# kepengxu/PGTFormer

Measured on NVIDIA H100. Metric: clips_per_s, higher is better.
Workload: dtype bf16

## Files before the change

include/pgt_b200.h:

```cpp
#ifndef PGT_B200_H_
#define PGT_B200_H_

#include <stdint.h>

#ifdef __cplusplus
extern "C" {
#endif

typedef enum pgt_status {
  PGT_OK = 0,
  PGT_ERR_INVALID = -1,
  PGT_ERR_CUDA = -2,
  PGT_ERR_UNSUPPORTED = -3,
  PGT_ERR_DRIVER = -4
} pgt_status;

enum { PGT_BF16 = 0, PGT_F32 = 1 };
enum { PGT_ACT_NONE = 0, PGT_ACT_GELU = 1, PGT_ACT_SILU = 2, PGT_ACT_LRELU02 = 3, PGT_ACT_RELU = 4,
       PGT_ACT_SIGMOID = 5 };
enum { PGT_EPI_PLAIN = 0,
       PGT_EPI_SFT = 1 };
enum { PGT_OUT_NHWC = 0, PGT_OUT_NCHW = 1 };
enum { PGT_EPI_FLAG_RELU_AFTER_RESIDUAL = 1 };

// ... 37 lines not shown

int pgt_conv_out_gn(const void* x, int F, int H, int W, int Cin, int ldx, const float* gn_ab, const void* Wp, int ldw,
                    int Cout, const float* bias, float* out, void* stream);
int pgt_conv_out_gn_act(const void* x, int F, int H, int W, int Cin, int ldx, const float* gn_ab, const void* Wp, int ldw,
                        int Cout, const float* bias, float* out, int silu, void* stream);

int pgt_conv_up2x_bf16(const void* x, int F, int Hin, int Win, int Cin, int ldx, const void* Wp4, int ldw,
                       int Cout, const pgt_epilogue* ep, void* stream);

int pgt_conv_rgb_bf16(const float* x_nchw, int F, int H, int W, int ksize, int stride, int pad, const float* mean3,
                      const float* std3, const void* Wp, int ldw, int Cout, const float* bias, int act, void* out,
                      int ldo, float* gn_stats, void* stream);

int64_t pgt_groupnorm_ws_floats(int F, int HW, int C);
int pgt_conv_tiles_per_frame(int Hin, int Win, int Cout, int ksize, int stride, int pad_lo);
int pgt_conv_tiles_exact(int Hin, int Win, int Cout, int ksize, int stride, int pad_lo);
int pgt_groupnorm_apply_stats(const void* x, int ldx, int F, int HW, int C, const float* gamma, const float* beta,
                              float eps, int apply_silu, void* y, int ldy, const float* stats, int chunks_per_frame,
                              float* ws, void* stream);

int pgt_groupnorm_ab(const void* x, int ldx, int F, int HW, int C, const float* gamma, const float* beta, float eps,
                     const float* stats, int chunks_per_frame, float* ws, float* ab, void* stream);
int pgt_groupnorm_silu(const void* x, int ldx, int F, int HW, int C, const float* gamma, const float* beta,
                       float eps, int apply_silu, void* y, int ldy, float* ws, void* stream);

int pgt_layernorm(const void* x, int ldx, int x_dtype, int T, int C, const float* gamma, const float* beta,
                  float eps, void* y, int ldy, const void* pos, int ldpos, void* y2, int ldy2, void* stream);

int pgt_ln_linear_bf16(const void* x, int ldx, int T, int C, const float* ln_g, const float* ln_b, float eps,
                       const void* W, int ldw, int N, const float* bias, void* out, int ldo, void* stream);

int pgt_swin_mlp_bf16(const void* x, int ldx, int T, int C, const float* ln_g, const float* ln_b, float eps,
                      const void* W1, const float* b1, const void* W2, const float* b2, void* out, int ldo,
                      float* gn_stats, void* stream);

int pgt_window_attention(const void* qkv, int ldqkv, int clips, int H, int W, int C, int heads, int shift,
                         const float* bias_tab, void* out, int ldo, void* stream);

int pgt_window_attention_tc(const void* qkv, int ldqkv, int clips, int H, int W, int C, int heads, int shift,
                            const void* tab, void* out, int ldo, void* stream);

int pgt_window3d_attention(const void* qkv, int ldqkv, const void* pad_qkv, int B, int D, int H, int W, int C, int heads,
                           int wd, int wh, int ww, int sd, int sh, int sw, const float* bias, void* out, int ldo,
                           void* stream);

int pgt_mha_fwd(const void* q, int ldq, const void* k, int ldk, const void* v, int ldv, int clips, int L,
                int heads, int d, void* out, int ldo, void* stream);

int pgt_argmax_gather(const float* logits, int T, int K, const float* codebook, int E, const int64_t* idx_in,
                      int64_t* idx, void* quant, int ldq, int quant_dtype, void* stream);
int pgt_l2_argmin(const float* z, int T, int E, const float* codebook, int K, int64_t* idx, float* quant,
                  void* stream);
int pgt_codebook_pack(const float* codebook, int K, int E, void* cb_bf16, float* cb_norm, void* stream);
int64_t pgt_l2_argmin_ws_ints(int T);
int pgt_l2_argmin_tc(const float* z, int T, int E, const float* codebook, const void* cb_bf16, const float* cb_norm,
                     int K, int64_t* idx, float* quant, int32_t* workspace, void* stream);
int64_t pgt_l2_argmin_split_ws_ints(int T, int splits);
int pgt_l2_argmin_tc_split(const float* z, int T, int E, const float* codebook, const void* cb_bf16, const float* cb_norm,
                           int K, int splits, int64_t* idx, float* quant, int32_t* workspace, void* stream);

int pgt_soft_codes(const float* z, int T, int E, const float* codebook, const float* cb_norm, int K, float temp,
                   float* out, int ldo, void* stream);
int pgt_sample_codes(const float* p, int T, int K, int ldp, const int64_t* seed, int64_t* idx, void* stream);

int pgt_rq_residual(const float* r_in, float* r_out, const int64_t* idx, int T, int E, const float* codebook_d,
                    float* agg, int first, void* stream);
int pgt_rq_embed(const int64_t* idx, long long ldi, long long ldd, int T, int d0, int d1, const float* codebooks,
// ... 35 lines not shown
```

pgtformer_b200/_lib.py:

```python
import ctypes
import os
from ctypes import POINTER, Structure, c_char_p, c_float, c_int, c_int32, c_int64, c_void_p

HERE = os.path.dirname(os.path.abspath(__file__))
LIB_PATH = os.path.join(HERE, 'lib', 'libpgt_b200.so')

BF16, F32 = 0, 1
ACT_NONE, ACT_GELU, ACT_SILU, ACT_LRELU02, ACT_RELU, ACT_SIGMOID = 0, 1, 2, 3, 4, 5
EPI_PLAIN, EPI_SFT = 0, 1
OUT_NHWC, OUT_NCHW = 0, 1


class Epilogue(Structure):
    _fields_ = [('bias', c_void_p), ('act', c_int32), ('mode', c_int32), ('residual', c_void_p),
                ('ldr', c_int32), ('res_dtype', c_int32), ('aux', c_void_p), ('ldaux', c_int32),
                ('sft_w', c_float), ('out', c_void_p), ('ldo', c_int32), ('out_dtype', c_int32),
                ('out_layout', c_int32), ('flags', c_int32), ('gn_stats', c_void_p), ('sft_wf', c_void_p)]


SIGNATURES = {
    'pgt_strerror': (c_char_p, [c_int]),
    'pgt_last_cuda_error': (c_char_p, []),
    'pgt_version': (c_int, []),
    'pgt_launch_count': (c_int64, []),
    'pgt_reset_launch_count': (None, []),
    'pgt_tmap_cache_stats': (None, [c_void_p, c_void_p]),
    'pgt_profile_begin': (c_int, []),
    'pgt_profile_end': (c_int, [c_void_p, c_void_p, c_void_p]),
    'pgt_profile_end_csv': (c_int, [c_char_p, c_void_p, c_void_p, c_void_p]),
    'pgt_linear_bf16': (c_int, [c_void_p, c_int, c_void_p, c_int, c_int, c_int, c_int, POINTER(Epilogue), c_void_p]),
    'pgt_conv_bf16': (c_int, [c_void_p, c_int, c_int, c_int, c_int, c_int, c_void_p, c_int, c_int, c_int, c_int,
                              c_int, POINTER(Epilogue), c_void_p]),
    'pgt_conv_out_gn': (c_int, [c_void_p, c_int, c_int, c_int, c_int, c_int, c_void_p, c_void_p, c_int, c_int, c_void_p,
                                c_void_p, c_void_p]),
    'pgt_conv_out_gn_act': (c_int, [c_void_p, c_int, c_int, c_int, c_int, c_int, c_void_p, c_void_p, c_int, c_int,
                                    c_void_p, c_void_p, c_int, c_void_p]),
    'pgt_groupnorm_ab': (c_int, [c_void_p, c_int, c_int, c_int, c_int, c_void_p, c_void_p, c_float, c_void_p, c_int,
                                 c_void_p, c_void_p, c_void_p]),
    'pgt_conv_up2x_bf16': (c_int, [c_void_p, c_int, c_int, c_int, c_int, c_int, c_void_p, c_int, c_int,
                                   POINTER(Epilogue), c_void_p]),
    'pgt_conv_rgb_bf16': (c_int, [c_void_p, c_int, c_int, c_int, c_int, c_int, c_int, c_void_p, c_void_p, c_void_p, c_int,
                                  c_int, c_void_p, c_int, c_void_p, c_int, c_void_p, c_void_p]),
    'pgt_groupnorm_ws_floats': (c_int64, [c_int, c_int, c_int]),
    'pgt_conv_tiles_per_frame': (c_int, [c_int, c_int, c_int, c_int, c_int, c_int]),
    'pgt_conv_tiles_exact': (c_int, [c_int, c_int, c_int, c_int, c_int, c_int]),
    'pgt_groupnorm_apply_stats': (c_int, [c_void_p, c_int, c_int, c_int, c_int, c_void_p, c_void_p, c_float, c_int,
                                          c_void_p, c_int, c_void_p, c_int, c_void_p, c_void_p]),
    'pgt_groupnorm_silu': (c_int, [c_void_p, c_int, c_int, c_int, c_int, c_void_p, c_void_p, c_float, c_int,
                                   c_void_p, c_int, c_void_p, c_void_p]),
    'pgt_layernorm': (c_int, [c_void_p, c_int, c_int, c_int, c_int, c_void_p, c_void_p, c_float, c_void_p, c_int,
                              c_void_p, c_int, c_void_p, c_int, c_void_p]),
    'pgt_ln_linear_bf16': (c_int, [c_void_p, c_int, c_int, c_int, c_void_p, c_void_p, c_float, c_void_p, c_int, c_int,
                                   c_void_p, c_void_p, c_int, c_void_p]),
    'pgt_swin_mlp_bf16': (c_int, [c_void_p, c_int, c_int, c_int, c_void_p, c_void_p, c_float, c_void_p, c_void_p, c_void_p,
                                  c_void_p, c_void_p, c_int, c_void_p, c_void_p]),
    'pgt_window_attention': (c_int, [c_void_p, c_int, c_int, c_int, c_int, c_int, c_int, c_int, c_void_p, c_void_p,
                                     c_int, c_void_p]),
    'pgt_window_attention_tc': (c_int, [c_void_p, c_int, c_int, c_int, c_int, c_int, c_int, c_int, c_void_p, c_void_p,
                                        c_int, c_void_p]),
    'pgt_window3d_attention': (c_int, [c_void_p, c_int, c_void_p, c_int, c_int, c_int, c_int, c_int, c_int, c_int, c_int,
                                       c_int, c_int, c_int, c_int, c_void_p, c_void_p, c_int, c_void_p]),
    'pgt_mha_fwd': (c_int, [c_void_p, c_int, c_void_p, c_int, c_void_p, c_int, c_int, c_int, c_int, c_int, c_void_p,
                            c_int, c_void_p]),
    'pgt_argmax_gather': (c_int, [c_void_p, c_int, c_int, c_void_p, c_int, c_void_p, c_void_p, c_void_p, c_int,
                                  c_int, c_void_p]),
    'pgt_l2_argmin': (c_int, [c_void_p, c_int, c_int, c_void_p, c_int, c_void_p, c_void_p, c_void_p]),
    'pgt_codebook_pack': (c_int, [c_void_p, c_int, c_int, c_void_p, c_void_p, c_void_p]),
    'pgt_l2_argmin_ws_ints': (c_int64, [c_int]),
    'pgt_l2_argmin_tc': (c_int, [c_void_p, c_int, c_int, c_void_p, c_void_p, c_void_p, c_int, c_void_p, c_void_p,
                                 c_void_p, c_void_p]),
    'pgt_l2_argmin_split_ws_ints': (c_int64, [c_int, c_int]),
    'pgt_l2_argmin_tc_split': (c_int, [c_void_p, c_int, c_int, c_void_p, c_void_p, c_void_p, c_int, c_int, c_void_p,
                                       c_void_p, c_void_p, c_void_p]),
    'pgt_soft_codes': (c_int, [c_void_p, c_int, c_int, c_void_p, c_void_p, c_int, c_float, c_void_p, c_int, c_void_p]),
    'pgt_sample_codes': (c_int, [c_void_p, c_int, c_int, c_int, c_void_p, c_void_p, c_void_p]),
    'pgt_rq_residual': (c_int, [c_void_p, c_void_p, c_void_p, c_int, c_int, c_void_p, c_void_p, c_int, c_void_p]),
    'pgt_rq_embed': (c_int, [c_void_p, c_int64, c_int64, c_int, c_int, c_int, c_void_p, c_int64, c_int, c_void_p, c_int,
                             c_int, c_void_p]),
    'pgt_vq_stats_ws_doubles': (c_int64, [c_int, c_int]),
    'pgt_vq_stats': (c_int, [c_void_p, c_int, c_int, c_int, c_void_p, c_int, c_void_p, c_float, c_void_p, c_void_p,
                             c_void_p, c_void_p, c_void_p, c_void_p, c_void_p, c_void_p, c_void_p]),
    'pgt_adain': (c_int, [c_void_p, c_int, c_int, c_void_p, c_int, c_int, c_int, c_int, c_float, c_void_p, c_int,
                          c_void_p]),
    'pgt_adain_frames': (c_int, [c_void_p, c_int, c_int, c_void_p, c_int, c_int, c_int, c_int, c_float, c_void_p,
                                 c_void_p, c_int, c_void_p]),
    'pgt_maxpool3x3s2': (c_int, [c_void_p, c_int, c_int, c_int, c_int, c_int, c_void_p, c_int, c_void_p]),
    'pgt_global_avgpool': (c_int, [c_void_p, c_int, c_int, c_int, c_int, c_void_p, c_int, c_void_p]),
    'pgt_channel_affine': (c_int, [c_void_p, c_int, c_int, c_int, c_int, c_void_p, c_int, c_int, c_void_p, c_int,
# ... 46 lines not shown
```

pgtformer_b200/csrc/swin_mlp.cu:

```cuda
#include <cudaTypedefs.h>

#include "common.cuh"
#include "tmap.cuh"
#include "ptx.cuh"
#include "epi_common.cuh"

namespace pgt {

constexpr int SM_C = 256;
constexpr int SM_BM = 128;
constexpr int SM_SUB = SM_BM * 128;
constexpr int SM_WST = 3;
constexpr int SM_WBYTES = SM_C * 128;
constexpr int SM_THREADS = 320;
constexpr int SM_XLD = 68;
constexpr int SM_XCH = SM_BM * SM_XLD * 4;
constexpr int SM_SMEM = 4 * SM_SUB  + SM_WST * SM_WBYTES + SM_XCH + 128 * 8  + 256;
static_assert(SM_SMEM <= 232448, "swin_mlp smem budget");

struct SwinMlpParams {
  int T, m_tiles;
  const float* ln_g;
  const float* ln_b;
  float eps;
  const float* b1;
  const float* b2;
  float* gn_stats;
};

struct SmBars {
  uint64_t x_full, res_full, acc2_done, out_ready;
};

__device__ __forceinline__ void swin_mlp_compute(const SwinMlpParams& p, uint8_t* sX, uint8_t* sW, float* xacc, float2* xln,
                                                 SmBars* bar, uint64_t* w_full, uint64_t* w_empty, int warp, int lane) {
  const int wg = warp >> 2, w = warp & 3;
  const int half = w >> 1;
  const int rl = (w & 1) * 32 + lane;
  const int r = wg * 64 + rl;
  const int quad = r >> 5;
  const int bar_id = 1 + wg;
  float* xw = xacc + wg * 64 * SM_XLD;
  const float* xrow = xw + rl * SM_XLD;
  const uint32_t a_rows = smem_u32(sX) + wg * 64 * 128;
  int st = 0;
  uint32_t ph = 0;
  uint32_t par = 0;
  float acc[SM_C / 2];

  auto gemm = [&]() {
    int prev = -1;
    for (int kb = 0; kb < 4; ++kb) {
      mbar_wait(&w_full[st], ph);
      const uint64_t da = wgmma_desc_k_sw128(a_rows + kb * SM_SUB);
      const uint64_t db = wgmma_desc_k_sw128(smem_u32(sW) + st * SM_WBYTES);
      wgmma_fence();
#pragma unroll
      for (int k = 0; k < 4; ++k) wgmma_bf16<SM_C>(acc, da + 2 * k, db + 2 * k, (kb | k) != 0 ? 1u : 0u);
      wgmma_commit();
      wgmma_wait<1>();
      if (prev >= 0) { __syncwarp(); if (lane == 0) mbar_arrive(&w_empty[prev]); }
      prev = st;
      if (++st == SM_WST) { st = 0; ph ^= 1; }
    }
    wgmma_wait<0>();
    __syncwarp();
    if (lane == 0) mbar_arrive(&w_empty[prev]);
  };
  auto exchange = [&](auto gc, uint32_t (&v)[32]) {
    constexpr int G = decltype(gc)::value;
    named_bar_sync(bar_id, 128);
    acc_to_smem<64 * G, 64>(acc, xw, SM_XLD, w, lane);
    named_bar_sync(bar_id, 128);
    smem_row_32(xrow + half * 32, v);
  };

  for (int tile = blockIdx.x; tile < p.m_tiles; tile += gridDim.x, par ^= 1) {
    mbar_wait(&bar->x_full, par);
    float s = 0.f, q = 0.f;
#pragma unroll
    for (int sub = 0; sub < 2; ++sub) {
      const uint8_t* src = sX + (half * 2 + sub) * SM_SUB + r * 128;
#pragma unroll
      for (int c = 0; c < 8; ++c) {
        const uint4 u = *reinterpret_cast<const uint4*>(src + ((c ^ (r & 7)) << 4));
        const float2 a = unpack_bf16x2(u.x), b = unpack_bf16x2(u.y), cc = unpack_bf16x2(u.z), d = unpack_bf16x2(u.w);
        s += (a.x + a.y) + (b.x + b.y) + (cc.x + cc.y) + (d.x + d.y);
        q += a.x * a.x + a.y * a.y + b.x * b.x + b.y * b.y + cc.x * cc.x + cc.y * cc.y + d.x * d.x + d.y * d.y;
      }
    }
    if (half == 0) xln[r] = make_float2(s, q);
    named_bar_sync(bar_id, 128);
    if (half == 1) {
      const float2 o = xln[r];
      s += o.x; q += o.y;
      xln[r] = make_float2(s, q);
    }
    named_bar_sync(bar_id, 128);
    if (half == 0) {
      const float2 o = xln[r];
      s = o.x; q = o.y;
    }
    const float mean = s * (1.f / SM_C);
    const float var = fmaxf(q * (1.f / SM_C) - mean * mean, 0.f);
    const float rstd = rsqrtf(var + p.eps);
    const float nm = -mean * rstd;
#pragma unroll
    for (int sub = 0; sub < 2; ++sub) {
      const int kb = half * 2 + sub;
      uint8_t* row = sX + kb * SM_SUB + r * 128;
#pragma unroll
      for (int c = 0; c < 8; ++c) {
        uint4* ptr = reinterpret_cast<uint4*>(row + ((c ^ (r & 7)) << 4));
        const uint4 u = *ptr;
        const float2 a = unpack_bf16x2(u.x), b = unpack_bf16x2(u.y), cc = unpack_bf16x2(u.z), d = unpack_bf16x2(u.w);
        const float v[8] = {a.x, a.y, b.x, b.y, cc.x, cc.y, d.x, d.y};
        float y[8];
        if (p.ln_g != nullptr) {
          const int col = kb * 64 + c * 8;
          const float4 g0 = __ldg(reinterpret_cast<const float4*>(p.ln_g + col)), g1 = __ldg(reinterpret_cast<const float4*>(p.ln_g + col + 4));
          const float4 e0 = __ldg(reinterpret_cast<const float4*>(p.ln_b + col)), e1 = __ldg(reinterpret_cast<const float4*>(p.ln_b + col + 4));
          const float gg[8] = {g0.x, g0.y, g0.z, g0.w, g1.x, g1.y, g1.z, g1.w};
          const float ee[8] = {e0.x, e0.y, e0.z, e0.w, e1.x, e1.y, e1.z, e1.w};
#pragma unroll
          for (int j = 0; j < 8; ++j) y[j] = fmaf(fmaf(v[j], rstd, nm), gg[j], ee[j]);
        } else {
#pragma unroll
          for (int j = 0; j < 8; ++j) y[j] = fmaf(v[j], rstd, nm);
        }
        uint4 o;
        o.x = pack_bf16x2(y[0], y[1]); o.y = pack_bf16x2(y[2], y[3]);
        o.z = pack_bf16x2(y[4], y[5]); o.w = pack_bf16x2(y[6], y[7]);
        *ptr = o;
      }
    }
    fence_proxy_async();
    named_bar_sync(bar_id, 128);
    gemm();
    static_for<0, SM_C / 64>([&](auto gc) {
      constexpr int G = decltype(gc)::value;
      uint32_t v[32];
      exchange(gc, v);
      const int c0 = G * 64 + half * 32;
      const float4* b4 = reinterpret_cast<const float4*>(p.b1 + c0);
      uint8_t* dst = sX + G * SM_SUB + r * 128;
      const int ch0 = half * 4;
#pragma unroll
      for (int i = 0; i < 4; ++i) {
        const float4 ba = __ldg(b4 + 2 * i), bb = __ldg(b4 + 2 * i + 1);
        uint4 o;
        o.x = pack_bf16x2(gelu_erf(__uint_as_float(v[8 * i + 0]) + ba.x), gelu_erf(__uint_as_float(v[8 * i + 1]) + ba.y));
        o.y = pack_bf16x2(gelu_erf(__uint_as_float(v[8 * i + 2]) + ba.z), gelu_erf(__uint_as_float(v[8 * i + 3]) + ba.w));
        o.z = pack_bf16x2(gelu_erf(__uint_as_float(v[8 * i + 4]) + bb.x), gelu_erf(__uint_as_float(v[8 * i + 5]) + bb.y));
        o.w = pack_bf16x2(gelu_erf(__uint_as_float(v[8 * i + 6]) + bb.z), gelu_erf(__uint_as_float(v[8 * i + 7]) + bb.w));
        *reinterpret_cast<uint4*>(dst + (((ch0 + i) ^ (r & 7)) << 4)) = o;
      }
    });
    fence_proxy_async();
    named_bar_sync(bar_id, 128);
    gemm();
    __syncwarp();
    if (lane == 0) mbar_arrive(&bar->acc2_done);
    mbar_wait(&bar->res_full, par);
    static_for<0, SM_C / 64>([&](auto gc) {
      constexpr int G = decltype(gc)::value;
      uint32_t v[32];
      exchange(gc, v);
      const int c0 = G * 64 + half * 32;
      float f[32];
      const float4* b4 = reinterpret_cast<const float4*>(p.b2 + c0);
      uint8_t* row = sX + G * SM_SUB + r * 128;
      const int ch0 = half * 4;
#pragma unroll
      for (int i = 0; i < 4; ++i) {
        const float4 ba = __ldg(b4 + 2 * i), bb = __ldg(b4 + 2 * i + 1);
        uint4* dst = reinterpret_cast<uint4*>(row + (((ch0 + i) ^ (r & 7)) << 4));
        const uint4 u = *dst;
        const float2 a = unpack_bf16x2(u.x), b = unpack_bf16x2(u.y), cc = unpack_bf16x2(u.z), d = unpack_bf16x2(u.w);
        f[8 * i + 0] = __uint_as_float(v[8 * i + 0]) + ba.x + a.x;  f[8 * i + 1] = __uint_as_float(v[8 * i + 1]) + ba.y + a.y;
        f[8 * i + 2] = __uint_as_float(v[8 * i + 2]) + ba.z + b.x;  f[8 * i + 3] = __uint_as_float(v[8 * i + 3]) + ba.w + b.y;
        f[8 * i + 4] = __uint_as_float(v[8 * i + 4]) + bb.x + cc.x; f[8 * i + 5] = __uint_as_float(v[8 * i + 5]) + bb.y + cc.y;
        f[8 * i + 6] = __uint_as_float(v[8 * i + 6]) + bb.z + d.x;  f[8 * i + 7] = __uint_as_float(v[8 * i + 7]) + bb.w + d.y;
        uint4 o;
        o.x = pack_bf16x2(f[8 * i + 0], f[8 * i + 1]); o.y = pack_bf16x2(f[8 * i + 2], f[8 * i + 3]);
        o.z = pack_bf16x2(f[8 * i + 4], f[8 * i + 5]); o.w = pack_bf16x2(f[8 * i + 6], f[8 * i + 7]);
        *dst = o;
      }
      if (p.gn_stats != nullptr)
        gn_chunk_stats<8>(f, p.gn_stats + (((size_t)tile * 4 + quad) * 32 + c0 / 8) * 2, 0, lane);
    });
    fence_proxy_async();
    mbar_arrive(&bar->out_ready);
  }
}

__global__ void __launch_bounds__(SM_THREADS, 1)
swin_mlp_kernel(const __grid_constant__ CUtensorMap tmX, const __grid_constant__ CUtensorMap tmO,
                const __grid_constant__ CUtensorMap tmW1, const __grid_constant__ CUtensorMap tmW2,
                const SwinMlpParams p) {
  extern __shared__ __align__(1024) uint8_t smem[];
  if ((smem_u32(smem) & 1023u) != 0) __trap();
  uint8_t* sX = smem;
  uint8_t* sW = smem + 4 * SM_SUB;
  float* xacc = reinterpret_cast<float*>(sW + SM_WST * SM_WBYTES);
  float2* xln = reinterpret_cast<float2*>(sW + SM_WST * SM_WBYTES + SM_XCH);
  SmBars* bar = reinterpret_cast<SmBars*>(xln + 128);
  uint64_t* w_full = reinterpret_cast<uint64_t*>(bar + 1);
  uint64_t* w_empty = w_full + SM_WST;

  const int warp = threadIdx.x >> 5, lane = threadIdx.x & 31;
  if (warp == 8 && lane == 0) {
    tma_prefetch_desc(&tmX); tma_prefetch_desc(&tmO); tma_prefetch_desc(&tmW1); tma_prefetch_desc(&tmW2);
    mbar_init(&bar->x_full, 1); mbar_init(&bar->res_full, 1);
    mbar_init(&bar->acc2_done, 8); mbar_init(&bar->out_ready, 256);
    for (int i = 0; i < SM_WST; ++i) { mbar_init(&w_full[i], 1); mbar_init(&w_empty[i], 8); }
    fence_barrier_init();
  }
  __syncthreads();

  if (warp == 8) {
    int st = 0;
    uint32_t ph = 0;
    for (int tile = blockIdx.x; tile < p.m_tiles; tile += gridDim.x) {
      for (int gemm = 0; gemm < 2; ++gemm) {
        for (int kb = 0; kb < 4; ++kb) {
          mbar_wait(&w_empty[st], ph ^ 1);
          if (elect_one()) {
            mbar_arrive_expect_tx(&w_full[st], SM_WBYTES);
            tma_load_2d(sW + st * SM_WBYTES, gemm == 0 ? &tmW1 : &tmW2, &w_full[st], kb * 64, 0);
          }
          __syncwarp();
          if (++st == SM_WST) { st = 0; ph ^= 1; }
        }
      }
    }
  } else if (warp == 9) {
    uint32_t par = 0;
    for (int tile = blockIdx.x; tile < p.m_tiles; tile += gridDim.x, par ^= 1) {
      if (lane == 0) {
        mbar_arrive_expect_tx(&bar->x_full, 4 * SM_SUB);
        for (int kb = 0; kb < 4; ++kb) tma_load_2d(sX + kb * SM_SUB, &tmX, &bar->x_full, kb * 64, tile * SM_BM);
      }
      __syncwarp();
      mbar_wait(&bar->acc2_done, par);
      if (lane == 0) {
        mbar_arrive_expect_tx(&bar->res_full, 4 * SM_SUB);
        for (int kb = 0; kb < 4; ++kb) tma_load_2d(sX + kb * SM_SUB, &tmX, &bar->res_full, kb * 64, tile * SM_BM);
      }
      __syncwarp();
      mbar_wait(&bar->out_ready, par);
      if (lane == 0) {
        for (int kb = 0; kb < 4; ++kb) tma_store_2d(&tmO, sX + kb * SM_SUB, kb * 64, tile * SM_BM);
        bulk_commit();
        bulk_wait_read<0>();
      }
      __syncwarp();
    }
    if (lane == 0) bulk_wait0();
  } else {
    swin_mlp_compute(p, sX, sW, xacc, xln, bar, w_full, w_empty, warp, lane);

  }
}

static int enc2d(CUtensorMap* map, const void* base, int ld, long long rows, int cols, int box_rows) {
  return tmap_rows_bf16(map, base, ld, rows, cols, box_rows);
}

}

using namespace pgt;

extern "C" int pgt_swin_mlp_bf16(const void* x, int ldx, int T, int C, const float* ln_g, const float* ln_b, float eps,
                                 const void* W1, const float* b1, const void* W2, const float* b2, void* out, int ldo,
                                 float* gn_stats, void* stream) {
  PGT_CHECK_ARG(x && out && W1 && W2 && b1 && b2 && T > 0 && ((ln_g == nullptr) == (ln_b == nullptr)));
  if (C != SM_C) return PGT_ERR_UNSUPPORTED;
  auto al = [](const void* q) { return (reinterpret_cast<uintptr_t>(q) & 15) == 0; };
  PGT_CHECK_ARG(al(x) && al(out) && al(W1) && al(W2) && ldx % 8 == 0 && ldo % 8 == 0);
  CUtensorMap tx, to, t1, t2;
  int rc = enc2d(&tx, x, ldx, T, C, SM_BM);
  if (rc == PGT_OK) rc = enc2d(&to, out, ldo, T, C, SM_BM);
  if (rc == PGT_OK) rc = enc2d(&t1, W1, C, C, C, SM_C);
  if (rc == PGT_OK) rc = enc2d(&t2, W2, C, C, C, SM_C);
  if (rc != PGT_OK) return rc;
  static PerDeviceOnce once;
  PGT_CUDA_OK(once.run([] { return cudaFuncSetAttribute(swin_mlp_kernel, cudaFuncAttributeMaxDynamicSharedMemorySize, SM_SMEM); }));
  SwinMlpParams p{};
  p.T = T; p.m_tiles = ceil_div(T, SM_BM);
  p.ln_g = ln_g; p.ln_b = ln_b; p.eps = eps; p.b1 = b1; p.b2 = b2; p.gn_stats = gn_stats;
  cudaStream_t st = static_cast<cudaStream_t>(stream);
  const int grid = p.m_tiles < num_sms() ? p.m_tiles : num_sms();
  {
    ProfScope ps(PGT_PROF_GEMM, 4.0 * (double)T * C * C, st, "swin_mlp_fused C256");
    swin_mlp_kernel<<<grid, SM_THREADS, SM_SMEM, st>>>(tx, to, t1, t2, p);
  }
  PGT_LAUNCH_OK();
  return PGT_OK;
}
```

pgtformer_b200/engine.py:

```python
import torch
import torch.nn.functional as F

from . import ops
from .spec import Arch
from .swin3d import pack_blocks

BF = torch.bfloat16


def _on_device(fn):
    import functools

    @functools.wraps(fn)
    def wrapper(self, *a, **k):
        with torch.cuda.device(self.dev):
            return fn(self, *a, **k)
    return wrapper


def _fusing(feats, wgt):
    return feats is not None and (torch.is_tensor(wgt) or wgt > 0)


def _pack_conv(w):
# ... 154 lines not shown
        if out is None:
            out = self._new(Fr, H // stride, W // stride, cout)
        stats = None
        if gn_out:
            stats = self._gn_stats(out, 4 * self._stats_tiles(H, W, cout, kw.get('ksize', 3), stride, kw.get('pad_lo', 1)),
                                   gn_into)
        return ops.conv(x, self.w[p + '.weight'], cout, out, bias=self.w.get(p + '.bias'), gn_stats=stats, **kw)

    def _lin(self, x, p, n, out=None, out_dtype=BF, gn_out=False, **kw):
        if out is None:
            out = self._new(*x.shape[:-1], n, dtype=out_dtype)
        stats = None
        if gn_out and out.dim() == 4 and out.dtype == BF and (out.shape[1] * out.shape[2]) % 128 == 0:
            stats = self._gn_stats(out, out.shape[1] * out.shape[2] // 32)
        return ops.linear(x, self.w[p + '.weight'], out, bias=self.w.get(p + '.bias'), N=n, gn_stats=stats, **kw)

    def td_resblock(self, x, p, cout, gn_next=False, out=None, shortcut='nin_shortcut'):
        h = self._conv3(x, p + '.conv1', cout, gn=p + '.norm1', gn_out=True)
        sc = self._lin(x, p + '.' + shortcut, cout) if (p + '.' + shortcut + '.weight') in self.w else x
        return self._conv3(h, p + '.conv2', cout, gn=p + '.norm2', residual=sc, gn_out=gn_next, out=out)

    def swin_block(self, x, p, heads, shift, gn_next=False, out=None):
        Fr, H, W, C = x.shape
        w = self.w
        if C == 256:
            qkv = ops.ln_linear(x, None, None, w[p + '.attn.qkv_ln.weight'], w[p + '.attn.qkv_ln.bias'],
                                self._new(Fr, H, W, 3 * C))
        else:
            y = ops.layernorm(x, w[p + '.norm1.weight'], w[p + '.norm1.bias'], self._new(Fr, H, W, C))
            qkv = self._lin(y, p + '.attn.qkv', 3 * C)
        a = self._new(Fr, H, W, C)
        if ops.window_attention_tc(qkv, Fr // 3, H, W, C, heads, shift, w[p + '.attn.tab16'], a) is None:
            ops.window_attention(qkv, Fr // 3, H, W, C, heads, shift, w[p + '.attn.bias_tab'], a)
        x = self._lin(a, p + '.attn.proj', C, residual=x)
        if C == 256:
            out = self._new(Fr, H, W, C) if out is None else out
            stats = self._gn_stats(out, H * W // 32) if gn_next and (H * W) % 128 == 0 else None
            return ops.swin_mlp(x, None, None, w[p + '.mlp.fc1_ln.weight'], w[p + '.mlp.fc1_ln.bias'],
                                w[p + '.mlp.fc2.weight'], w[p + '.mlp.fc2.bias'], out, gn_stats=stats)
        y = ops.layernorm(x, w[p + '.norm2.weight'], w[p + '.norm2.bias'], self._new(Fr, H, W, C))
        m = self._lin(y, p + '.mlp.fc1', C, act=ops.ACT_GELU)
        return self._lin(m, p + '.mlp.fc2', C, residual=x, gn_out=gn_next, out=out)

    def attn_block(self, x, p, gn_next=False):
        Fr, H, W, C = x.shape
        y = self._gn(x, p + '.norm', silu=False)
        qkv = self._lin(y, p + '.qkv', 3 * C)
        a = ops.mha(qkv[..., :C], qkv[..., C:2 * C], qkv[..., 2 * C:], Fr, H * W, 1, C, self._new(Fr, H, W, C))
        return self._lin(a, p + '.proj_out', C, residual=x, gn_out=gn_next)

    def encoder_layer(self, x, p, heads, depth, gn_next=False, out=None):
        for i in range(depth):
            x = self.swin_block(x, '%s.blocks.%d' % (p, i), heads, 2 if i % 2 == 1 else 0,
                                gn_next=gn_next and i == depth - 1, out=out if i == depth - 1 else None)
        return x

    def _cat_slot(self, Fr, H, W, C):
        return self._new(Fr, H, W, 2 * C + 32)

    def fuse_sft(self, enc, dec, key, wgt, gn_next=False):
        p = 'fuse_convs_dict.' + key
        Fr, H, W, C = dec.shape
        b, P = Fr // 3, H * W
        cat = getattr(enc, '_pgt_cat', None)
        if cat is None or getattr(dec, '_pgt_cat', None) is not cat:
            cat = self._new(Fr, H, W, 2 * C + 32)
            ops.copy2d(enc, cat[..., :C])
            ops.copy2d(dec, cat[..., C:2 * C])
        tcat = self._new(b, P, 192)
        ops.regroup_frames(self._lin(enc, p + '.tconvenc', 32), tcat[..., :96], b, P, 32, 0)
        ops.regroup_frames(self._lin(dec, p + '.tconvdec', 32), tcat[..., 96:], b, P, 32, 0)
        fut = ops.regroup_frames(self._lin(tcat, p + '.tfusion0', 96), self._new(Fr, P, 32), b, P, 32, 1)
# ... 540 lines not shown
```

pgtformer_b200/ops.py:

```python
import ctypes

import torch

from . import _lib as L
from ._lib import (ACT_GELU, ACT_LRELU02, ACT_NONE, ACT_RELU, ACT_SIGMOID, ACT_SILU, BF16, EPI_PLAIN,
                   EPI_SFT, F32, OUT_NCHW, OUT_NHWC, Epilogue)


def _p(t):
    return ctypes.c_void_p(t.data_ptr()) if t is not None else None


def _stream(t=None):
    if t is not None:
        return ctypes.c_void_p(torch.cuda.current_stream(t.device).cuda_stream)
    return ctypes.c_void_p(torch.cuda.current_stream().cuda_stream)


def _dt(t):
    if t.dtype == torch.bfloat16:
        return BF16
    if t.dtype == torch.float32:
        return F32
    raise TypeError('unsupported dtype %s' % t.dtype)
# ... 162 lines not shown
    assert x.dtype == torch.bfloat16 and x.stride(3) == 1 and x.stride(1) == W * x.stride(2) and \
        (F == 1 or x.stride(0) == H * x.stride(1))
    assert out.dtype == torch.float32 and out.is_contiguous() and tuple(out.shape) == (F, cout, H, W)
    if silu:
        rc = lib.pgt_conv_out_gn(_p(x), F, H, W, Cin, x.stride(2), _p(ab), _p(wp), wp.stride(0), cout, _p(bias), _p(out),
                                 _stream(x))
    else:
        rc = lib.pgt_conv_out_gn_act(_p(x), F, H, W, Cin, x.stride(2), _p(ab), _p(wp), wp.stride(0), cout, _p(bias),
                                     _p(out), 0, _stream(x))
    if rc == -3:
        return None
    L.check(rc)
    return out


def layernorm(x, gamma, beta, out, eps=1e-5, pos=None, out2=None):
    lib = L.load()
    T, C, ldx = _rows(x)
    L.check(lib.pgt_layernorm(_p(x), ldx, _dt(x), T, C, _p(gamma), _p(beta), eps, _p(out), _rows(out)[2],
                              _p(pos), _rows(pos)[2] if pos is not None else 0,
                              _p(out2), _rows(out2)[2] if out2 is not None else 0, _stream()))
    return out


def ln_linear(x, ln_g, ln_b, w, bias, out, eps=1e-5):
    lib = L.load()
    T, C, ldx = _rows(x)
    assert x.dtype == torch.bfloat16 and w.dtype == torch.bfloat16 and w.stride(1) == 1 and out.dtype == torch.bfloat16
    L.check(lib.pgt_ln_linear_bf16(_p(x), ldx, T, C, _p(ln_g), _p(ln_b), eps, _p(w), w.stride(0), w.shape[0], _p(bias),
                                   _p(out), _rows(out)[2], _stream()))
    return out


def swin_mlp(x, ln_g, ln_b, w1, b1, w2, b2, out, eps=1e-5, gn_stats=None):
    lib = L.load()
    T, C, ldx = _rows(x)
    assert x.dtype == torch.bfloat16 and w1.dtype == torch.bfloat16 and w1.is_contiguous() and w2.is_contiguous()
    L.check(lib.pgt_swin_mlp_bf16(_p(x), ldx, T, C, _p(ln_g), _p(ln_b), eps, _p(w1), _p(b1), _p(w2), _p(b2), _p(out),
                                  _rows(out)[2], _p(gn_stats), _stream()))
    return out


def window_attention(qkv, clips, H, W, C, heads, shift, bias_tab, out):
    lib = L.load()
    assert qkv.dtype == torch.bfloat16 and bias_tab.dtype == torch.float32 and bias_tab.is_contiguous()
    L.check(lib.pgt_window_attention(_p(qkv), _rows(qkv)[2], clips, H, W, C, heads, shift, _p(bias_tab), _p(out),
                                     _rows(out)[2], _stream()))
    return out


LOG2E = 1.4426950408889634


def window_tables(bias):
    heads = bias.shape[0]
    dev = bias.device
    r = torch.arange(48, device=dev)
    tabs = []
    for t in range(4):
        if t == 0:
            f, iy, ix = r // 16, (r // 4) % 4, r % 4
        elif t == 1:
            rr = r % 24
            f, iy, ix = rr // 8, (rr % 8) // 2, rr % 2 + 2 * (r // 24)
        elif t == 2:
            rr = r % 24
            f, iy, ix = rr // 8, (rr % 8) // 4 + 2 * (r // 24), rr % 4
        else:
            pp, rr = r // 12, r % 12
            f, iy, ix = rr // 4, (rr % 4) // 2 + 2 * (pp // 2), rr % 2 + 2 * (pp % 2)
        canon = f * 16 + iy * 4 + ix
        tt = bias[:, canon][:, :, canon].float() * LOG2E
# ... 312 lines not shown
```

Measured before the change: 90.05.

## Fuse attention output projection with residual into the Swin MLP kernel

For C=256 Swin blocks, the attention projection GEMM, its bias and the residual add now run inside the fused MLP kernel. The kernel loads the attention output as the GEMM A operand and the block input as the residual. It stages the projected result in a second shared buffer that serves as both the LN source and the MLP residual. This removes a separate linear launch and the global round trip of the intermediate x. In exchange the weight pipeline shrinks to 2 stages to fit the larger shared-memory footprint, and the kernel carries more work per tile.

Result: no change. 90.69, median of 6 (+0.7%).

```diff
diff --git a/include/pgt_b200.h b/include/pgt_b200.h
--- a/include/pgt_b200.h
+++ b/include/pgt_b200.h
@@ -93,7 +93,7 @@
 
 int pgt_swin_mlp_bf16(const void* x, int ldx, int T, int C, const float* ln_g, const float* ln_b, float eps,
                       const void* W1, const float* b1, const void* W2, const float* b2, void* out, int ldo,
-                      float* gn_stats, void* stream);
+                      float* gn_stats, const void* a, int lda, const void* Wp, const float* bp, void* stream);
 
 int pgt_window_attention(const void* qkv, int ldqkv, int clips, int H, int W, int C, int heads, int shift,
                          const float* bias_tab, void* out, int ldo, void* stream);
diff --git a/pgtformer_b200/_lib.py b/pgtformer_b200/_lib.py
--- a/pgtformer_b200/_lib.py
+++ b/pgtformer_b200/_lib.py
@@ -53,7 +53,7 @@
     'pgt_ln_linear_bf16': (c_int, [c_void_p, c_int, c_int, c_int, c_void_p, c_void_p, c_float, c_void_p, c_int, c_int,
                                    c_void_p, c_void_p, c_int, c_void_p]),
     'pgt_swin_mlp_bf16': (c_int, [c_void_p, c_int, c_int, c_int, c_void_p, c_void_p, c_float, c_void_p, c_void_p, c_void_p,
-                                  c_void_p, c_void_p, c_int, c_void_p, c_void_p]),
+                                  c_void_p, c_void_p, c_int, c_void_p, c_void_p, c_int, c_void_p, c_void_p, c_void_p]),
     'pgt_window_attention': (c_int, [c_void_p, c_int, c_int, c_int, c_int, c_int, c_int, c_int, c_void_p, c_void_p,
                                      c_int, c_void_p]),
     'pgt_window_attention_tc': (c_int, [c_void_p, c_int, c_int, c_int, c_int, c_int, c_int, c_int, c_void_p, c_void_p,
diff --git a/pgtformer_b200/csrc/swin_mlp.cu b/pgtformer_b200/csrc/swin_mlp.cu
--- a/pgtformer_b200/csrc/swin_mlp.cu
+++ b/pgtformer_b200/csrc/swin_mlp.cu
@@ -15,8 +15,13 @@
 constexpr int SM_THREADS = 320;
 constexpr int SM_XLD = 68;
 constexpr int SM_XCH = SM_BM * SM_XLD * 4;
-constexpr int SM_SMEM = 4 * SM_SUB  + SM_WST * SM_WBYTES + SM_XCH + 128 * 8  + 256;
-static_assert(SM_SMEM <= 232448, "swin_mlp smem budget");
+template <bool kProj> constexpr int sm_wst() { return kProj ? 2 : SM_WST; }
+template <bool kProj>
+constexpr int sm_smem() {
+  return (kProj ? 8 : 4) * SM_SUB  + sm_wst<kProj>() * SM_WBYTES + SM_XCH +
+         (kProj ? 0 : 128 * 8)  + 256;
+}
+static_assert(sm_smem<false>() <= 232448 && sm_smem<true>() <= 232448, "swin_mlp smem budget");
 
 struct SwinMlpParams {
   int T, m_tiles;
@@ -26,14 +31,18 @@
   const float* b1;
   const float* b2;
   float* gn_stats;
+  const float* bp;
 };
 
 struct SmBars {
   uint64_t x_full, res_full, acc2_done, out_ready;
 };
 
-__device__ __forceinline__ void swin_mlp_compute(const SwinMlpParams& p, uint8_t* sX, uint8_t* sW, float* xacc, float2* xln,
-                                                 SmBars* bar, uint64_t* w_full, uint64_t* w_empty, int warp, int lane) {
+template <bool kProj>
+__device__ __forceinline__ void swin_mlp_compute(const SwinMlpParams& p, uint8_t* sX, uint8_t* sR, uint8_t* sW, float* xacc,
+                                                 float2* xln, SmBars* bar, uint64_t* w_full, uint64_t* w_empty, int warp,
+                                                 int lane) {
+  constexpr int WST = sm_wst<kProj>();
   const int wg = warp >> 2, w = warp & 3;
   const int half = w >> 1;
   const int rl = (w & 1) * 32 + lane;
@@ -42,6 +51,7 @@
   const int bar_id = 1 + wg;
   float* xw = xacc + wg * 64 * SM_XLD;
   const float* xrow = xw + rl * SM_XLD;
+  float2* xln_r = kProj ? reinterpret_cast<float2*>(xacc + r * SM_XLD + 64) : xln + r;
   const uint32_t a_rows = smem_u32(sX) + wg * 64 * 128;
   int st = 0;
   uint32_t ph = 0;
@@ -61,7 +71,7 @@
       wgmma_wait<1>();
       if (prev >= 0) { __syncwarp(); if (lane == 0) mbar_arrive(&w_empty[prev]); }
       prev = st;
-      if (++st == SM_WST) { st = 0; ph ^= 1; }
+      if (++st == WST) { st = 0; ph ^= 1; }
     }
     wgmma_wait<0>();
     __syncwarp();
@@ -75,12 +85,48 @@
     smem_row_32(xrow + half * 32, v);
   };
 
+  auto residual_epi = [&](auto gc, const float* bias, uint8_t* buf, float* gn, int tile) {
+    constexpr int G = decltype(gc)::value;
+    uint32_t v[32];
+    exchange(gc, v);
+    const int c0 = G * 64 + half * 32;
+    float f[32];
+    const float4* b4 = reinterpret_cast<const float4*>(bias + c0);
+    uint8_t* row = buf + G * SM_SUB + r * 128;
+    const int ch0 = half * 4;
+#pragma unroll
+    for (int i = 0; i < 4; ++i) {
+      const float4 ba = __ldg(b4 + 2 * i), bb = __ldg(b4 + 2 * i + 1);
+      uint4* dst = reinterpret_cast<uint4*>(row + (((ch0 + i) ^ (r & 7)) << 4));
+      const uint4 u = *dst;
+      const float2 a = unpack_bf16x2(u.x), b = unpack_bf16x2(u.y), cc = unpack_bf16x2(u.z), d = unpack_bf16x2(u.w);
+      f[8 * i + 0] = __uint_as_float(v[8 * i + 0]) + ba.x + a.x;  f[8 * i + 1] = __uint_as_float(v[8 * i + 1]) + ba.y + a.y;
+      f[8 * i + 2] = __uint_as_float(v[8 * i + 2]) + ba.z + b.x;  f[8 * i + 3] = __uint_as_float(v[8 * i + 3]) + ba.w + b.y;
+      f[8 * i + 4] = __uint_as_float(v[8 * i + 4]) + bb.x + cc.x; f[8 * i + 5] = __uint_as_float(v[8 * i + 5]) + bb.y + cc.y;
+      f[8 * i + 6] = __uint_as_float(v[8 * i + 6]) + bb.z + d.x;  f[8 * i + 7] = __uint_as_float(v[8 * i + 7]) + bb.w + d.y;
+      uint4 o;
+      o.x = pack_bf16x2(f[8 * i + 0], f[8 * i + 1]); o.y = pack_bf16x2(f[8 * i + 2], f[8 * i + 3]);
+      o.z = pack_bf16x2(f[8 * i + 4], f[8 * i + 5]); o.w = pack_bf16x2(f[8 * i + 6], f[8 * i + 7]);
+      *dst = o;
+    }
+    if (gn != nullptr)
+      gn_chunk_stats<8>(f, gn + (((size_t)tile * 4 + quad) * 32 + c0 / 8) * 2, 0, lane);
+  };
+
   for (int tile = blockIdx.x; tile < p.m_tiles; tile += gridDim.x, par ^= 1) {
     mbar_wait(&bar->x_full, par);
+    uint8_t* sO = sX;
+    if constexpr (kProj) {
+      gemm();
+      mbar_wait(&bar->res_full, par);
+      static_for<0, SM_C / 64>([&](auto gc) { residual_epi(gc, p.bp, sR, nullptr, tile); });
+      named_bar_sync(bar_id, 128);
+      sO = sR;
+    }
     float s = 0.f, q = 0.f;
 #pragma unroll
     for (int sub = 0; sub < 2; ++sub) {
-      const uint8_t* src = sX + (half * 2 + sub) * SM_SUB + r * 128;
+      const uint8_t* src = sO + (half * 2 + sub) * SM_SUB + r * 128;
 #pragma unroll
       for (int c = 0; c < 8; ++c) {
         const uint4 u = *reinterpret_cast<const uint4*>(src + ((c ^ (r & 7)) << 4));
@@ -89,16 +135,16 @@
         q += a.x * a.x + a.y * a.y + b.x * b.x + b.y * b.y + cc.x * cc.x + cc.y * cc.y + d.x * d.x + d.y * d.y;
       }
     }
-    if (half == 0) xln[r] = make_float2(s, q);
+    if (half == 0) *xln_r = make_float2(s, q);
     named_bar_sync(bar_id, 128);
     if (half == 1) {
-      const float2 o = xln[r];
+      const float2 o = *xln_r;
       s += o.x; q += o.y;
-      xln[r] = make_float2(s, q);
+      *xln_r = make_float2(s, q);
     }
     named_bar_sync(bar_id, 128);
     if (half == 0) {
-      const float2 o = xln[r];
+      const float2 o = *xln_r;
       s = o.x; q = o.y;
     }
     const float mean = s * (1.f / SM_C);
@@ -108,11 +154,12 @@
 #pragma unroll
     for (int sub = 0; sub < 2; ++sub) {
       const int kb = half * 2 + sub;
+      const uint8_t* srow = sO + kb * SM_SUB + r * 128;
       uint8_t* row = sX + kb * SM_SUB + r * 128;
 #pragma unroll
       for (int c = 0; c < 8; ++c) {
         uint4* ptr = reinterpret_cast<uint4*>(row + ((c ^ (r & 7)) << 4));
-        const uint4 u = *ptr;
+        const uint4 u = *reinterpret_cast<const uint4*>(srow + ((c ^ (r & 7)) << 4));
         const float2 a = unpack_bf16x2(u.x), b = unpack_bf16x2(u.y), cc = unpack_bf16x2(u.z), d = unpack_bf16x2(u.w);
         const float v[8] = {a.x, a.y, b.x, b.y, cc.x, cc.y, d.x, d.y};
         float y[8];
@@ -161,59 +208,37 @@
     gemm();
     __syncwarp();
     if (lane == 0) mbar_arrive(&bar->acc2_done);
-    mbar_wait(&bar->res_full, par);
-    static_for<0, SM_C / 64>([&](auto gc) {
-      constexpr int G = decltype(gc)::value;
-      uint32_t v[32];
-      exchange(gc, v);
-      const int c0 = G * 64 + half * 32;
-      float f[32];
-      const float4* b4 = reinterpret_cast<const float4*>(p.b2 + c0);
-      uint8_t* row = sX + G * SM_SUB + r * 128;
-      const int ch0 = half * 4;
-#pragma unroll
-      for (int i = 0; i < 4; ++i) {
-        const float4 ba = __ldg(b4 + 2 * i), bb = __ldg(b4 + 2 * i + 1);
-        uint4* dst = reinterpret_cast<uint4*>(row + (((ch0 + i) ^ (r & 7)) << 4));
-        const uint4 u = *dst;
-        const float2 a = unpack_bf16x2(u.x), b = unpack_bf16x2(u.y), cc = unpack_bf16x2(u.z), d = unpack_bf16x2(u.w);
-        f[8 * i + 0] = __uint_as_float(v[8 * i + 0]) + ba.x + a.x;  f[8 * i + 1] = __uint_as_float(v[8 * i + 1]) + ba.y + a.y;
-        f[8 * i + 2] = __uint_as_float(v[8 * i + 2]) + ba.z + b.x;  f[8 * i + 3] = __uint_as_float(v[8 * i + 3]) + ba.w + b.y;
-        f[8 * i + 4] = __uint_as_float(v[8 * i + 4]) + bb.x + cc.x; f[8 * i + 5] = __uint_as_float(v[8 * i + 5]) + bb.y + cc.y;
-        f[8 * i + 6] = __uint_as_float(v[8 * i + 6]) + bb.z + d.x;  f[8 * i + 7] = __uint_as_float(v[8 * i + 7]) + bb.w + d.y;
-        uint4 o;
-        o.x = pack_bf16x2(f[8 * i + 0], f[8 * i + 1]); o.y = pack_bf16x2(f[8 * i + 2], f[8 * i + 3]);
-        o.z = pack_bf16x2(f[8 * i + 4], f[8 * i + 5]); o.w = pack_bf16x2(f[8 * i + 6], f[8 * i + 7]);
-        *dst = o;
-      }
-      if (p.gn_stats != nullptr)
-        gn_chunk_stats<8>(f, p.gn_stats + (((size_t)tile * 4 + quad) * 32 + c0 / 8) * 2, 0, lane);
-    });
+    if constexpr (!kProj) mbar_wait(&bar->res_full, par);
+    static_for<0, SM_C / 64>([&](auto gc) { residual_epi(gc, p.b2, sO, p.gn_stats, tile); });
     fence_proxy_async();
     mbar_arrive(&bar->out_ready);
   }
 }
 
+template <bool kProj>
 __global__ void __launch_bounds__(SM_THREADS, 1)
 swin_mlp_kernel(const __grid_constant__ CUtensorMap tmX, const __grid_constant__ CUtensorMap tmO,
                 const __grid_constant__ CUtensorMap tmW1, const __grid_constant__ CUtensorMap tmW2,
-                const SwinMlpParams p) {
+                const SwinMlpParams p, const __grid_constant__ CUtensorMap tmA, const __grid_constant__ CUtensorMap tmP) {
+  constexpr int WST = sm_wst<kProj>();
   extern __shared__ __align__(1024) uint8_t smem[];
   if ((smem_u32(smem) & 1023u) != 0) __trap();
   uint8_t* sX = smem;
-  uint8_t* sW = smem + 4 * SM_SUB;
-  float* xacc = reinterpret_cast<float*>(sW + SM_WST * SM_WBYTES);
-  float2* xln = reinterpret_cast<float2*>(sW + SM_WST * SM_WBYTES + SM_XCH);
-  SmBars* bar = reinterpret_cast<SmBars*>(xln + 128);
+  uint8_t* sR = smem + 4 * SM_SUB;
+  uint8_t* sW = smem + (kProj ? 8 : 4) * SM_SUB;
+  float* xacc = reinterpret_cast<float*>(sW + WST * SM_WBYTES);
+  float2* xln = reinterpret_cast<float2*>(sW + WST * SM_WBYTES + SM_XCH);
+  SmBars* bar = reinterpret_cast<SmBars*>(kProj ? reinterpret_cast<uint8_t*>(xln) : reinterpret_cast<uint8_t*>(xln + 128));
   uint64_t* w_full = reinterpret_cast<uint64_t*>(bar + 1);
-  uint64_t* w_empty = w_full + SM_WST;
+  uint64_t* w_empty = w_full + WST;
 
   const int warp = threadIdx.x >> 5, lane = threadIdx.x & 31;
   if (warp == 8 && lane == 0) {
     tma_prefetch_desc(&tmX); tma_prefetch_desc(&tmO); tma_prefetch_desc(&tmW1); tma_prefetch_desc(&tmW2);
+    if constexpr (kProj) { tma_prefetch_desc(&tmA); tma_prefetch_desc(&tmP); }
     mbar_init(&bar->x_full, 1); mbar_init(&bar->res_full, 1);
     mbar_init(&bar->acc2_done, 8); mbar_init(&bar->out_ready, 256);
-    for (int i = 0; i < SM_WST; ++i) { mbar_init(&w_full[i], 1); mbar_init(&w_empty[i], 8); }
+    for (int i = 0; i < WST; ++i) { mbar_init(&w_full[i], 1); mbar_init(&w_empty[i], 8); }
     fence_barrier_init();
   }
   __syncthreads();
@@ -222,18 +247,48 @@
     int st = 0;
     uint32_t ph = 0;
     for (int tile = blockIdx.x; tile < p.m_tiles; tile += gridDim.x) {
-      for (int gemm = 0; gemm < 2; ++gemm) {
+      for (int gemm = kProj ? -1 : 0; gemm < 2; ++gemm) {
         for (int kb = 0; kb < 4; ++kb) {
           mbar_wait(&w_empty[st], ph ^ 1);
           if (elect_one()) {
             mbar_arrive_expect_tx(&w_full[st], SM_WBYTES);
-            tma_load_2d(sW + st * SM_WBYTES, gemm == 0 ? &tmW1 : &tmW2, &w_full[st], kb * 64, 0);
+            tma_load_2d(sW + st * SM_WBYTES, gemm < 0 ? &tmP : gemm == 0 ? &tmW1 : &tmW2, &w_full[st], kb * 64, 0);
           }
           __syncwarp();
-          if (++st == SM_WST) { st = 0; ph ^= 1; }
+          if (++st == WST) { st = 0; ph ^= 1; }
         }
       }
     }
+  } else if (kProj && warp == 9) {
+    uint32_t par = 0;
+    if (lane == 0 && (int)blockIdx.x < p.m_tiles) {
+      mbar_arrive_expect_tx(&bar->x_full, 4 * SM_SUB);
+      for (int kb = 0; kb < 4; ++kb) tma_load_2d(sX + kb * SM_SUB, &tmA, &bar->x_full, kb * 64, blockIdx.x * SM_BM);
+      mbar_arrive_expect_tx(&bar->res_full, 4 * SM_SUB);
+      for (int kb = 0; kb < 4; ++kb) tma_load_2d(sR + kb * SM_SUB, &tmX, &bar->res_full, kb * 64, blockIdx.x * SM_BM);
+    }
+    __syncwarp();
+    for (int tile = blockIdx.x; tile < p.m_tiles; tile += gridDim.x, par ^= 1) {
+      const int next = tile + gridDim.x;
+      mbar_wait(&bar->acc2_done, par);
+      if (lane == 0 && next < p.m_tiles) {
+        mbar_arrive_expect_tx(&bar->x_full, 4 * SM_SUB);
+        for (int kb = 0; kb < 4; ++kb) tma_load_2d(sX + kb * SM_SUB, &tmA, &bar->x_full, kb * 64, next * SM_BM);
+      }
+      __syncwarp();
+      mbar_wait(&bar->out_ready, par);
+      if (lane == 0) {
+        for (int kb = 0; kb < 4; ++kb) tma_store_2d(&tmO, sR + kb * SM_SUB, kb * 64, tile * SM_BM);
+        bulk_commit();
+        bulk_wait_read<0>();
+        if (next < p.m_tiles) {
+          mbar_arrive_expect_tx(&bar->res_full, 4 * SM_SUB);
+          for (int kb = 0; kb < 4; ++kb) tma_load_2d(sR + kb * SM_SUB, &tmX, &bar->res_full, kb * 64, next * SM_BM);
+        }
+      }
+      __syncwarp();
+    }
+    if (lane == 0) bulk_wait0();
   } else if (warp == 9) {
     uint32_t par = 0;
     for (int tile = blockIdx.x; tile < p.m_tiles; tile += gridDim.x, par ^= 1) {
@@ -258,7 +313,7 @@
     }
     if (lane == 0) bulk_wait0();
   } else {
-    swin_mlp_compute(p, sX, sW, xacc, xln, bar, w_full, w_empty, warp, lane);
+    swin_mlp_compute<kProj>(p, sX, sR, sW, xacc, xln, bar, w_full, w_empty, warp, lane);
 
   }
 }
@@ -273,27 +328,41 @@
 
 extern "C" int pgt_swin_mlp_bf16(const void* x, int ldx, int T, int C, const float* ln_g, const float* ln_b, float eps,
                                  const void* W1, const float* b1, const void* W2, const float* b2, void* out, int ldo,
-                                 float* gn_stats, void* stream) {
+                                 float* gn_stats, const void* a, int lda, const void* Wp, const float* bp, void* stream) {
   PGT_CHECK_ARG(x && out && W1 && W2 && b1 && b2 && T > 0 && ((ln_g == nullptr) == (ln_b == nullptr)));
+  const bool proj = a != nullptr;
+  PGT_CHECK_ARG((Wp == nullptr) == !proj && (bp == nullptr) == !proj);
   if (C != SM_C) return PGT_ERR_UNSUPPORTED;
   auto al = [](const void* q) { return (reinterpret_cast<uintptr_t>(q) & 15) == 0; };
   PGT_CHECK_ARG(al(x) && al(out) && al(W1) && al(W2) && ldx % 8 == 0 && ldo % 8 == 0);
-  CUtensorMap tx, to, t1, t2;
+  PGT_CHECK_ARG(!proj || (al(a) && al(Wp) && lda % 8 == 0));
+  CUtensorMap tx, to, t1, t2, ta, tp;
   int rc = enc2d(&tx, x, ldx, T, C, SM_BM);
   if (rc == PGT_OK) rc = enc2d(&to, out, ldo, T, C, SM_BM);
   if (rc == PGT_OK) rc = enc2d(&t1, W1, C, C, C, SM_C);
   if (rc == PGT_OK) rc = enc2d(&t2, W2, C, C, C, SM_C);
+  if (rc == PGT_OK && proj) rc = enc2d(&ta, a, lda, T, C, SM_BM);
+  if (rc == PGT_OK && proj) rc = enc2d(&tp, Wp, C, C, C, SM_C);
   if (rc != PGT_OK) return rc;
-  static PerDeviceOnce once;
-  PGT_CUDA_OK(once.run([] { return cudaFuncSetAttribute(swin_mlp_kernel, cudaFuncAttributeMaxDynamicSharedMemorySize, SM_SMEM); }));
   SwinMlpParams p{};
   p.T = T; p.m_tiles = ceil_div(T, SM_BM);
-  p.ln_g = ln_g; p.ln_b = ln_b; p.eps = eps; p.b1 = b1; p.b2 = b2; p.gn_stats = gn_stats;
+  p.ln_g = ln_g; p.ln_b = ln_b; p.eps = eps; p.b1 = b1; p.b2 = b2; p.gn_stats = gn_stats; p.bp = bp;
   cudaStream_t st = static_cast<cudaStream_t>(stream);
   const int grid = p.m_tiles < num_sms() ? p.m_tiles : num_sms();
-  {
+  if (proj) {
+    static PerDeviceOnce once;
+    PGT_CUDA_OK(once.run([] {
+      return cudaFuncSetAttribute(swin_mlp_kernel<true>, cudaFuncAttributeMaxDynamicSharedMemorySize, sm_smem<true>());
+    }));
+    ProfScope ps(PGT_PROF_GEMM, 6.0 * (double)T * C * C, st, "swin_mlp_fused proj C256");
+    swin_mlp_kernel<true><<<grid, SM_THREADS, sm_smem<true>(), st>>>(tx, to, t1, t2, p, ta, tp);
+  } else {
+    static PerDeviceOnce once;
+    PGT_CUDA_OK(once.run([] {
+      return cudaFuncSetAttribute(swin_mlp_kernel<false>, cudaFuncAttributeMaxDynamicSharedMemorySize, sm_smem<false>());
+    }));
     ProfScope ps(PGT_PROF_GEMM, 4.0 * (double)T * C * C, st, "swin_mlp_fused C256");
-    swin_mlp_kernel<<<grid, SM_THREADS, SM_SMEM, st>>>(tx, to, t1, t2, p);
+    swin_mlp_kernel<false><<<grid, SM_THREADS, sm_smem<false>(), st>>>(tx, to, t1, t2, p, tx, t1);
   }
   PGT_LAUNCH_OK();
   return PGT_OK;
diff --git a/pgtformer_b200/engine.py b/pgtformer_b200/engine.py
--- a/pgtformer_b200/engine.py
+++ b/pgtformer_b200/engine.py
@@ -210,12 +210,13 @@
         a = self._new(Fr, H, W, C)
         if ops.window_attention_tc(qkv, Fr // 3, H, W, C, heads, shift, w[p + '.attn.tab16'], a) is None:
             ops.window_attention(qkv, Fr // 3, H, W, C, heads, shift, w[p + '.attn.bias_tab'], a)
-        x = self._lin(a, p + '.attn.proj', C, residual=x)
         if C == 256:
             out = self._new(Fr, H, W, C) if out is None else out
             stats = self._gn_stats(out, H * W // 32) if gn_next and (H * W) % 128 == 0 else None
             return ops.swin_mlp(x, None, None, w[p + '.mlp.fc1_ln.weight'], w[p + '.mlp.fc1_ln.bias'],
-                                w[p + '.mlp.fc2.weight'], w[p + '.mlp.fc2.bias'], out, gn_stats=stats)
+                                w[p + '.mlp.fc2.weight'], w[p + '.mlp.fc2.bias'], out, gn_stats=stats,
+                                attn=a, proj_w=w[p + '.attn.proj.weight'], proj_b=w[p + '.attn.proj.bias'])
+        x = self._lin(a, p + '.attn.proj', C, residual=x)
         y = ops.layernorm(x, w[p + '.norm2.weight'], w[p + '.norm2.bias'], self._new(Fr, H, W, C))
         m = self._lin(y, p + '.mlp.fc1', C, act=ops.ACT_GELU)
         return self._lin(m, p + '.mlp.fc2', C, residual=x, gn_out=gn_next, out=out)
diff --git a/pgtformer_b200/ops.py b/pgtformer_b200/ops.py
--- a/pgtformer_b200/ops.py
+++ b/pgtformer_b200/ops.py
@@ -218,12 +218,21 @@
     return out
 
 
-def swin_mlp(x, ln_g, ln_b, w1, b1, w2, b2, out, eps=1e-5, gn_stats=None):
+def swin_mlp(x, ln_g, ln_b, w1, b1, w2, b2, out, eps=1e-5, gn_stats=None, attn=None, proj_w=None, proj_b=None):
     lib = L.load()
     T, C, ldx = _rows(x)
     assert x.dtype == torch.bfloat16 and w1.dtype == torch.bfloat16 and w1.is_contiguous() and w2.is_contiguous()
+    lda = 0
+    if attn is not None:
+        assert proj_w is not None and proj_b is not None
+        assert attn.dtype == torch.bfloat16 and proj_w.dtype == torch.bfloat16 and proj_w.is_contiguous()
+        assert proj_b.dtype == torch.float32 and proj_b.is_contiguous()
+        Ta, Ca, lda = _rows(attn)
+        assert (Ta, Ca) == (T, C)
+    else:
+        assert proj_w is None and proj_b is None
     L.check(lib.pgt_swin_mlp_bf16(_p(x), ldx, T, C, _p(ln_g), _p(ln_b), eps, _p(w1), _p(b1), _p(w2), _p(b2), _p(out),
-                                  _rows(out)[2], _p(gn_stats), _stream()))
+                                  _rows(out)[2], _p(gn_stats), _p(attn), lda, _p(proj_w), _p(proj_b), _stream()))
     return out
 
 
```
